# beecave-homelab/VibeVoice-ROCm

Hardware: AMD Instinct MI355X
Metric: audio-sec/s (higher is better)
Workload: dtype bf16; 1 GPU; cfg2: VibeVoice-1.5B shapes, 1 speaker(s) x 203-frame voice prompt, 330-token prompt, 225 frames (30.0 s audio), CFG=2.0, 20 DPM-Solver++ steps, whole generate() incl. voice encode + prefill; global_batch=1, parallelism=replicas x1 (one dialogue per GPU), hipgraph=True

## Files before the change

vibevoice_rocm_amd/csrc/vv_common.h:

```cpp
#ifndef VV_COMMON_H
#define VV_COMMON_H
#include <hip/hip_runtime.h>
#include <stdarg.h>
#include <stdint.h>
#include "vv_hip.h"

int vv_set_error(int code, const char* fmt, ...);

#define VV_CHECK_LAUNCH(name)                                                                    \
  do {                                                                                           \
    hipError_t e_ = hipGetLastError();                                                           \
    if (e_ != hipSuccess) return vv_set_error(VV_E_HIP, "%s: %s", name, hipGetErrorString(e_));  \
  } while (0)

#define VV_TRY(expr)            \
  do {                          \
    int rc_ = (expr);           \
    if (rc_) return rc_;        \
  } while (0)

struct vv_kv_args {
  void* k; void* v;
  int kvdt, layers, rows, kv_heads, s_max, head_dim;
  void* vt;
  vv_kv_args(const vv_kv& a) : k(a.k), v(a.v), kvdt(a.kvdt), layers(a.layers), rows(a.rows), kv_heads(a.kv_heads), s_max(a.s_max), head_dim(a.head_dim), vt(a.vt) {}
};
struct vv_kv_args8 : vv_kv_args {
  const float* kscale; const float* vscale;
  vv_kv_args8(const vv_kv& a) : vv_kv_args(a), kscale(a.kscale), vscale(a.vscale) {}
};

int vv_launch_gemv_stream(const vv_lin_args& a, hipStream_t s);
struct vv_gemv_hot_shape { const char* name; int m, n, k, dual, pro, mod, bias, gate, res, act, flags; };
extern "C" int vv_gemv_hot_shapes(vv_gemv_hot_shape* out, int cap);
int vv_launch_gemv_hot(const vv_lin_args& a, hipStream_t s);
void vv_gemv_hot_set(int mask);
int vv_launch_conv_hot_gemv(const vv_lin_args& a, hipStream_t s);
int vv_launch_conv_hot_row(const vv_block& B, const float* x, float* y, float* hidden, float* hist_new, int C, float eps, hipStream_t s);
void vv_conv_hot_set(int mask);
int vv_launch_gemv_rows(const vv_lin_args& a, float* part, size_t part_floats, int* tickets, size_t n_tickets, hipStream_t s);
size_t vv_gemv_rows_part_floats(int n, int dual);
size_t vv_gemv_rows_tickets(int n);
int vv_gemv_rows_init();
void vv_gemv_rows_set(int on, int blocks, int pers);
int vv_linear_ws(const vv_lin_args* a, const void* f1, const void* f2, float* part, size_t part_floats, int* tickets, size_t n_tickets,
                 vv_stream_t stream, const vv_w8* q1 = nullptr, const vv_w8* q2 = nullptr);
int vv_launch_mfma_gemm(const vv_lin_args& a, hipStream_t s);
int vv_mfma_gemm_init();
int vv_launch_attn_decode(const float* qkv, int64_t ld_qkv, int R, int heads, const vv_kv* kv, int layer, const float2* rope, const int* lens, float* out,
                          int64_t ldo, float* part, int* tickets, int nsplit, int part_cap, hipStream_t s);
int vv_attn_decode_ws(const float* qkv, int64_t ld_qkv, int R, int heads, const vv_kv* kv, int layer, const float* rope_table, const int* lens, float* out,
                      int64_t ldo, float* part, int* tickets, int nsplit, int part_cap, vv_stream_t stream);
int vv_launch_kv_quantize(const vv_kv* src, const vv_kv* dst, int src_row, int dst_row, int len, int flags, hipStream_t s);
int vv_launch_attn_prefill(const float* qkv, int64_t ld_qkv, int R, int heads, const vv_kv* kv, int layer, const int* lens, const int* cache_rows,
                           float* out, int64_t ldo, hipStream_t s);
int vv_head_init_fused(const vv_head* h, const float* noise, float* Xs, float* Ms, float* h0, int64_t ldh, hipStream_t s);
bool vv_head_boundary_supported(const vv_head* h);
int vv_head_boundary_fused(const vv_head* h, const float* hrows, int64_t ldh, const float* shift, const float* scale, int64_t ld_mod, float cfg,
                           const vv_dpm_coef* k, float* Xs, float* Ms, float* h_out, int64_t ldh_out, float* latent_out, hipStream_t s);
int vv_head_boundary_batch(const vv_head* h, const float* hrows, int64_t ldh, const float* shift, const float* scale, int64_t ld_mod, float cfg,
                           const vv_dpm_coef* k, float* Xs, float* Ms, int64_t state_stride, float* h_out, int64_t ldh_out, float* latent_out,
                           int64_t latent_stride, int B, hipStream_t s,
// ... 130 lines not shown
```

vibevoice_rocm_amd/csrc/vv_fused.hip:

```cpp
#include <hip/hip_runtime.h>
#include <stdint.h>

#include "vv_hip.h"
#include "vv_common.h"

namespace {

typedef unsigned short bf16_t;
__device__ __forceinline__ float bf2f(bf16_t v) { return __uint_as_float((unsigned)v << 16); }
__device__ __forceinline__ float ldw(const float* p) { return *p; }
__device__ __forceinline__ float ldw(const bf16_t* p) { return bf2f(*p); }

template <typename WT>
__global__ __launch_bounds__(256) void head_init_kernel(const WT* P, const float* noise, int D, int latent, float* Xs, float* Ms, float* h0, int64_t ldh) {
  extern __shared__ float nz[];
  for (int i = threadIdx.x; i < latent; i += blockDim.x) nz[i] = noise[i];
  __syncthreads();
  const int n = blockIdx.x * blockDim.x + threadIdx.x;
  if (n >= D + latent) return;
  float s;
  if (n < D) {
    s = 0.f;
    const WT* pr = P + (int64_t)n * latent;
    for (int j = 0; j < latent; ++j) s = fmaf(ldw(pr + j), nz[j], s);
// ... 146 lines not shown
    if (lane == 0) {
      const float x0 = a.k.alpha_s * xs_cur - a.k.sigma_s * z;
      float xt = a.k.cx * xs_cur - a.k.cd * x0;
      if (a.k.order == 2) xt -= 0.5f * a.k.cd * (a.k.rinv * (x0 - ms_cur));
      if constexpr (SDE) xt = fmaf(a.k.cn, nx_cur, xt);
      a.Xs[g] = xt;
      a.Ms[g] = x0;
      if (g < D) { a.h_out[g] = xt; a.h_out[a.ldh_out + g] = xt; }
      else a.latent_out[g - D] = xt;
    }
    g += gstride;
#pragma unroll
    for (int u = 0; u < KU; ++u) { cur[u][0] = nxt[u][0]; cur[u][1] = nxt[u][1]; }
    xs_cur = xs_nxt; ms_cur = ms_nxt;
    if constexpr (SDE) nx_cur = nx_nxt;
    if (g + gstride < N) {
      xs_nxt = a.Xs[g + gstride]; ms_nxt = a.Ms[g + gstride];
      if constexpr (SDE) nx_nxt = a.nx[g + gstride];
      issue(nxt, g + gstride);
    }
  }
}

template <int KU> void launch_boundary(const BoundaryArgs& a, int B, hipStream_t s) {
  const int n = a.D + a.latent;
  int blocks = (n + 3) / 4;
  if (blocks > 512) blocks = 512;
  if (B > 1 && blocks > 256) blocks = 256;
  if (a.nx) hipLaunchKernelGGL((head_boundary_kernel<KU, true>), dim3(blocks, B), dim3(256), 0, s, a);
  else hipLaunchKernelGGL((head_boundary_kernel<KU, false>), dim3(blocks, B), dim3(256), 0, s, a);
}

template <typename WT, bool SAMPLE>
__global__ __launch_bounds__(256) void llm_tail_kernel(const float* h, int64_t ldh, int R, int H, const float* norm_w, float eps, float* out, int64_t ldo,
                                                       const WT* w_valid, int nv, const int* ids, float* logits_out, int* token_out, const int* forced,
                                                       int* lens, int tok_start, int tok_diff, int* frame_ctr, const vv_sampler smp, const float* q) {
  extern __shared__ float hn0[];
  __shared__ float red[4];
  __shared__ float lg[16];
  const int tid = threadIdx.x, lane = tid & 63, wave = tid >> 6;
  for (int r = 0; r < R; ++r) {
    const float* xr = h + (int64_t)r * ldh;
    float s = 0.f;
    for (int c = tid; c < H; c += 256) { const float v = xr[c]; s = fmaf(v, v, s); }
    s = vv_wave_sum(s);
    __syncthreads();
    if (lane == 0) red[wave] = s;
    __syncthreads();
// ... 525 lines not shown
#pragma unroll
    for (int o = 0; o < 2; ++o)
#pragma unroll
      for (int r = 0; r < 2; ++r) c0[o][r] = vv_wave_sum(acc[o][r]);
#pragma unroll
    for (int ps = 0; ps < 2; ++ps) {
      const int i = lane + 64 * ps;
      if (i < a.n_steps) {
#pragma unroll
        for (int r = 0; r < 2; ++r) {
          const float v0 = c0[0][r] + te[ps][0], v1 = c0[1][r] + te[ps][1];
          const float s0 = v0 / (1.0f + expf(-v0)), s1 = v1 / (1.0f + expf(-v1));
          const unsigned u0 = __float_as_uint(s0), u1 = __float_as_uint(s1);
          const unsigned pk = ((u0 + 0x7fffu + ((u0 >> 16) & 1u)) >> 16) | (((u1 + 0x7fffu + ((u1 >> 16) & 1u)) >> 16) << 16);
          *reinterpret_cast<unsigned*>(a.c_out + ((int64_t)(i * 2 + r)) * D + n) = pk;
        }
      }
    }
  }
}

}

int vv_head_init_fused(const vv_head* h, const float* noise, float* Xs, float* Ms, float* h0, int64_t ldh, hipStream_t s) {
  const int n = h->D + h->latent;
  const int blocks = (n + 255) / 256;
  const size_t lds = (size_t)h->latent * sizeof(float);
  if (h->wdt == VV_F32) hipLaunchKernelGGL((head_init_kernel<float>), dim3(blocks), dim3(256), lds, s, (const float*)h->noisy_proj, noise, h->D, h->latent, Xs, Ms, h0, ldh);
  else hipLaunchKernelGGL((head_init_kernel<bf16_t>), dim3(blocks), dim3(256), lds, s, (const bf16_t*)h->noisy_proj, noise, h->D, h->latent, Xs, Ms, h0, ldh);
  VV_CHECK_LAUNCH("vv_head_init_fused");
  return 0;
}

int vv_head_sde_proj_fused(const vv_head* h, const float* sde_noise, int64_t ld_sde, int n_steps, int B, float* NX, hipStream_t s) {
  const int n = h->D + h->latent;
  const dim3 grid((n + 255) / 256, B * n_steps);
  const size_t lds = (size_t)h->latent * sizeof(float);
  if (h->wdt == VV_F32)
    hipLaunchKernelGGL((head_sde_proj_kernel<float>), grid, dim3(256), lds, s, (const float*)h->noisy_proj, sde_noise, ld_sde, n_steps, h->D, h->latent, NX);
  else
    hipLaunchKernelGGL((head_sde_proj_kernel<bf16_t>), grid, dim3(256), lds, s, (const bf16_t*)h->noisy_proj, sde_noise, ld_sde, n_steps, h->D, h->latent, NX);
  VV_CHECK_LAUNCH("vv_head_sde_proj_fused");
  return 0;
}

bool vv_head_boundary_supported(const vv_head* h) {
// ... 214 lines not shown
```

vibevoice_rocm_amd/csrc/vv_gemv_hot.hip:

```cpp
#include <hip/hip_runtime.h>
#include <stdint.h>

#include "vv_hip.h"
#include "vv_common.h"

namespace {

typedef unsigned short bf16_t;
typedef unsigned int u32x4 __attribute__((ext_vector_type(4)));
typedef float vf2 __attribute__((ext_vector_type(2)));

__device__ __forceinline__ float silu1(float v) { return v / (1.0f + expf(-v)); }

__device__ __forceinline__ void unpack8(const u32x4 v, float (&o)[8]) {
  o[0] = __uint_as_float(v.x << 16); o[1] = __uint_as_float(v.x & 0xffff0000u);
  o[2] = __uint_as_float(v.y << 16); o[3] = __uint_as_float(v.y & 0xffff0000u);
  o[4] = __uint_as_float(v.z << 16); o[5] = __uint_as_float(v.z & 0xffff0000u);
  o[6] = __uint_as_float(v.w << 16); o[7] = __uint_as_float(v.w & 0xffff0000u);
}

template <bool NT>
__device__ __forceinline__ u32x4 ldw(const bf16_t* p) {
  const u32x4* q = reinterpret_cast<const u32x4*>(p);
  if constexpr (NT) return __builtin_nontemporal_load(q);
  else return *q;
}

__device__ __forceinline__ void fma_unit(const u32x4 wv, const float (&x0)[8], const float (&x1)[8], vf2& p0, vf2& p1) {
  float w[8];
  unpack8(wv, w);
#pragma unroll
  for (int j = 0; j < 8; j += 2) p0 = __builtin_elementwise_fma(vf2{w[j], w[j + 1]}, vf2{x0[j], x0[j + 1]}, p0);
#pragma unroll
  for (int j = 0; j < 8; j += 2) p1 = __builtin_elementwise_fma(vf2{w[j], w[j + 1]}, vf2{x1[j], x1[j + 1]}, p1);
}

__device__ __forceinline__ float vv_hot_gate_res(float v, float g, float r) {
#pragma clang fp contract(off)
  const float t = v * g;
  return t + r;
}

#define VV_FENCE4(v) asm volatile("" : "+v"((v).x), "+v"((v).y), "+v"((v).z), "+v"((v).w))

template <int N, bool MOD, bool NT>
__global__ __launch_bounds__(256, 2) void hot_dual_kernel(const vv_lin_args a) {
  constexpr int K = 1536, KU = 3, M = 2, T = 256, NCH = 2, NCHUNKS = K / 4;
  constexpr int WAVES = 512 * 4, G = (N + WAVES - 1) / WAVES;
  constexpr bool RAGGED = (N % WAVES) != 0;
  __shared__ float red[4 * M];
  __shared__ __attribute__((aligned(16))) float xs[M * KU * 512];
  const int tid = threadIdx.x, lane = tid & 63;
  const int wave = __builtin_amdgcn_readfirstlane(tid >> 6);
  const int gw = wave * 512 + (int)blockIdx.x;
  const bf16_t* __restrict__ W = reinterpret_cast<const bf16_t*>(a.w);
  const bf16_t* __restrict__ W2 = reinterpret_cast<const bf16_t*>(a.w2);

  float4 xv[M][NCH], nv[NCH], sv[M][NCH], cv[M][NCH];
#pragma unroll
  for (int c = 0; c < NCH; ++c) {
    const int ch = tid + c * T;
    const int kk = ch < NCHUNKS ? ch * 4 : 0;
#pragma unroll
    for (int m = 0; m < M; ++m) xv[m][c] = *reinterpret_cast<const float4*>(a.x + (int64_t)m * a.ldx + kk);
    nv[c] = *reinterpret_cast<const float4*>(a.norm_w + kk);
    if constexpr (MOD) {
#pragma unroll
      for (int m = 0; m < M; ++m) {
        const int64_t mo = (int64_t)m * a.ld_mod + kk;
        sv[m][c] = *reinterpret_cast<const float4*>(a.mod_shift + mo);
        cv[m][c] = *reinterpret_cast<const float4*>(a.mod_scale + mo);
      }
    }
  }
  u32x4 wq[G][KU], wq2[G][KU];
#pragma unroll
  for (int i = 0; i < G; ++i) {
    const int n = gw + i * WAVES;
    const bool live = !RAGGED || i < G - 1 || n < N;
    const int off = live ? n * K + lane * 8 : 0;
#pragma unroll
    for (int u = 0; u < KU; ++u) {
      wq[i][u] = ldw<NT>(W + off + (live ? u * 512 : 0));
      wq2[i][u] = ldw<NT>(W2 + off + (live ? u * 512 : 0));
    }
  }
  __builtin_amdgcn_sched_barrier(0);
#pragma unroll
  for (int c = 0; c < NCH; ++c) {
#pragma unroll
    for (int m = 0; m < M; ++m) VV_FENCE4(xv[m][c]);
    VV_FENCE4(nv[c]);
    if constexpr (MOD) {
#pragma unroll
      for (int m = 0; m < M; ++m) { VV_FENCE4(sv[m][c]); VV_FENCE4(cv[m][c]); }
    }
  }

  float ss[M];
#pragma unroll
  for (int m = 0; m < M; ++m) {
    float s1 = 0.f;
#pragma unroll
    for (int c = 0; c < NCH; ++c) {
      const float4 v = xv[m][c];
      s1 += (tid + c * T < NCHUNKS) ? (v.x * v.x + v.y * v.y) + (v.z * v.z + v.w * v.w) : 0.f;
    }
    ss[m] = vv_wave_sum(s1);
  }
  if (lane == 0) {
#pragma unroll
    for (int m = 0; m < M; ++m) red[wave * M + m] = ss[m];
  }
  __syncthreads();
#pragma unroll
  for (int m = 0; m < M; ++m) {
    float tot = 0.f;
#pragma unroll
    for (int w4 = 0; w4 < 4; ++w4) tot += red[w4 * M + m];
    const float rstd = rsqrtf(tot / (float)a.k + a.eps);
#pragma unroll
    for (int c = 0; c < NCH; ++c) {
      const int ch = tid + c * T;
      float4 v = xv[m][c];
      v.x *= rstd; v.y *= rstd; v.z *= rstd; v.w *= rstd;
      v.x *= nv[c].x; v.y *= nv[c].y; v.z *= nv[c].z; v.w *= nv[c].w;
      if constexpr (MOD) {
        v.x = v.x * (1.0f + cv[m][c].x) + sv[m][c].x; v.y = v.y * (1.0f + cv[m][c].y) + sv[m][c].y;
        v.z = v.z * (1.0f + cv[m][c].z) + sv[m][c].z; v.w = v.w * (1.0f + cv[m][c].w) + sv[m][c].w;
      }
      if (ch < NCHUNKS) *reinterpret_cast<float4*>(&xs[(m * KU * 128 + ch) * 4]) = v;
    }
  }
  __syncthreads();
  float xr[M][KU][8];
#pragma unroll
  for (int m = 0; m < M; ++m)
#pragma unroll
    for (int u = 0; u < KU; ++u) {
      const float4 p = *reinterpret_cast<const float4*>(&xs[m * KU * 512 + u * 512 + lane * 8]);
      const float4 q = *reinterpret_cast<const float4*>(&xs[m * KU * 512 + u * 512 + lane * 8 + 4]);
      xr[m][u][0] = p.x; xr[m][u][1] = p.y; xr[m][u][2] = p.z; xr[m][u][3] = p.w;
      xr[m][u][4] = q.x; xr[m][u][5] = q.y; xr[m][u][6] = q.z; xr[m][u][7] = q.w;
    }

#pragma unroll
  for (int i = 0; i < G; ++i) {
    const int n = gw + i * WAVES;
    if (RAGGED && i == G - 1 && n >= N) break;
    vf2 p[M] = {vf2{0.f, 0.f}, vf2{0.f, 0.f}}, p2[M] = {vf2{0.f, 0.f}, vf2{0.f, 0.f}};
#pragma unroll
    for (int u = 0; u < KU; ++u) {
      fma_unit(wq[i][u], xr[0][u], xr[1][u], p[0], p[1]);
      fma_unit(wq2[i][u], xr[0][u], xr[1][u], p2[0], p2[1]);
    }
    float acc[M], acc2[M];
#pragma unroll
    for (int m = 0; m < M; ++m) {
      acc[m] = vv_wave_sum(p[m].x + p[m].y);
      acc2[m] = vv_wave_sum(p2[m].x + p2[m].y);
    }
    if (lane < M) {
      const float v = lane == 0 ? acc[0] : acc[1], v2 = lane == 0 ? acc2[0] : acc2[1];
      a.out[(int64_t)lane * a.ldo + n] = silu1(v) * v2;
    }
  }
}

template <int N, int WPB, bool RMS, bool NT>
__global__ __launch_bounds__(64 * WPB) void hot_rows_kernel(const vv_lin_args a) {
  constexpr int K = 1536, KU = 3, M = 2, RW = 2;
  static_assert(N % (RW * WPB) == 0, "every wave of the grid owns one whole row pair");
  const int tid = threadIdx.x, lane = tid & 63;
  const int wave = __builtin_amdgcn_readfirstlane(tid >> 6);
  const int g = (int)blockIdx.x * WPB + wave;
  const bf16_t* __restrict__ W = reinterpret_cast<const bf16_t*>(a.w);

  float4 xa[M][KU], xb[M][KU], na[KU], nb[KU];
#pragma unroll
  for (int m = 0; m < M; ++m) {
    const float* xrow = a.x + (int64_t)m * a.ldx + lane * 8;
#pragma unroll
    for (int u = 0; u < KU; ++u) {
      xa[m][u] = *reinterpret_cast<const float4*>(xrow + u * 512);
      xb[m][u] = *reinterpret_cast<const float4*>(xrow + u * 512 + 4);
    }
  }
  if constexpr (RMS) {
#pragma unroll
    for (int u = 0; u < KU; ++u) {
      na[u] = *reinterpret_cast<const float4*>(a.norm_w + u * 512 + lane * 8);
      nb[u] = *reinterpret_cast<const float4*>(a.norm_w + u * 512 + lane * 8 + 4);
    }
  }
  const int eo_id = lane < RW * M ? lane : 0;
  const int eo_r = eo_id >> 1, eo_m = eo_id & 1;
  const int eo_n = g * RW + eo_r;
  float eo;
  if constexpr (RMS) eo = a.bias[eo_n];
  else eo = a.res[(int64_t)eo_m * a.ldres + eo_n];
  u32x4 wq[RW][KU];
#pragma unroll
  for (int r = 0; r < RW; ++r)
#pragma unroll
    for (int u = 0; u < KU; ++u) wq[r][u] = ldw<NT>(W + (g * RW + r) * K + u * 512 + lane * 8);
  __builtin_amdgcn_sched_barrier(0);
#pragma unroll
  for (int u = 0; u < KU; ++u) {
#pragma unroll
    for (int m = 0; m < M; ++m) { VV_FENCE4(xa[m][u]); VV_FENCE4(xb[m][u]); }
    if constexpr (RMS) { VV_FENCE4(na[u]); VV_FENCE4(nb[u]); }
  }

  float xr[M][KU][8];
  float ss[M];
#pragma unroll
  for (int m = 0; m < M; ++m) {
    ss[m] = 0.f;
#pragma unroll
    for (int u = 0; u < KU; ++u) {
      xr[m][u][0] = xa[m][u].x; xr[m][u][1] = xa[m][u].y; xr[m][u][2] = xa[m][u].z; xr[m][u][3] = xa[m][u].w;
      xr[m][u][4] = xb[m][u].x; xr[m][u][5] = xb[m][u].y; xr[m][u][6] = xb[m][u].z; xr[m][u][7] = xb[m][u].w;
      if constexpr (RMS) {
#pragma unroll
        for (int j = 0; j < 8; ++j) ss[m] = fmaf(xr[m][u][j], xr[m][u][j], ss[m]);
      }
    }
  }
  if constexpr (RMS) {
#pragma unroll
    for (int m = 0; m < M; ++m) ss[m] = vv_wave_sum(ss[m]);
#pragma unroll
    for (int m = 0; m < M; ++m) {
      const float rstd = rsqrtf(ss[m] / (float)a.k + a.eps);
// ... 12 lines not shown

  vf2 p[RW][M];
#pragma unroll
  for (int r = 0; r < RW; ++r) {
    p[r][0] = vf2{0.f, 0.f}; p[r][1] = vf2{0.f, 0.f};
#pragma unroll
    for (int u = 0; u < KU; ++u) fma_unit(wq[r][u], xr[0][u], xr[1][u], p[r][0], p[r][1]);
  }
  float acc[RW][M];
#pragma unroll
  for (int r = 0; r < RW; ++r)
#pragma unroll
    for (int m = 0; m < M; ++m) acc[r][m] = vv_wave_sum(p[r][m].x + p[r][m].y);
  if (lane < RW * M) {
    const float v0 = (lane & 1) ? acc[0][1] : acc[0][0], v1 = (lane & 1) ? acc[1][1] : acc[1][0];
    float v = (lane & 2) ? v1 : v0;
    v += eo;
    a.out[(int64_t)eo_m * a.ldo + eo_n] = v;
  }
}

template <int N, int K, int R, bool GATE, bool NT>
__global__ __launch_bounds__(256) void hot_down_kernel(const vv_lin_args a) {
  constexpr int M = 2, NW = 4, UNITS = (K + 511) / 512, KU = (UNITS + NW - 1) / NW;
  static_assert(N % R == 0 && R * M <= 64, "whole row sets; the epilogue threads are the first R * M of the block");
  __shared__ float part[NW][R * M];
  const int tid = threadIdx.x, lane = tid & 63;
  const int wave = __builtin_amdgcn_readfirstlane(tid >> 6);
  const int n0 = (int)blockIdx.x * R;
  const bf16_t* __restrict__ W = reinterpret_cast<const bf16_t*>(a.w);

  int koff[KU];
  bool kval[KU];
#pragma unroll
  for (int u = 0; u < KU; ++u) {
    koff[u] = (wave + NW * u) * 512 + lane * 8;
    kval[u] = koff[u] < K;
    if (!kval[u]) koff[u] = 0;
  }
  float4 xa[M][KU], xb[M][KU];
#pragma unroll
  for (int m = 0; m < M; ++m) {
    const float* xrow = a.x + (int64_t)m * a.ldx;
#pragma unroll
    for (int u = 0; u < KU; ++u) {
      xa[m][u] = *reinterpret_cast<const float4*>(xrow + koff[u]);
// ... 7 lines not shown
  if constexpr (GATE) eg = a.gate[(int64_t)eo_m * a.gate_ld + eo_n];
  const float er = a.res[(int64_t)eo_m * a.ldres + eo_n];
  u32x4 wq[R][KU];
#pragma unroll
  for (int r = 0; r < R; ++r)
#pragma unroll
    for (int u = 0; u < KU; ++u) wq[r][u] = ldw<NT>(W + (n0 + r) * K + koff[u]);
  __builtin_amdgcn_sched_barrier(0);
#pragma unroll
  for (int u = 0; u < KU; ++u)
#pragma unroll
    for (int m = 0; m < M; ++m) { VV_FENCE4(xa[m][u]); VV_FENCE4(xb[m][u]); }

  float xr[M][KU][8];
#pragma unroll
  for (int m = 0; m < M; ++m)
#pragma unroll
    for (int u = 0; u < KU; ++u) {
      const bool kv = kval[u];
      xr[m][u][0] = kv ? xa[m][u].x : 0.f; xr[m][u][1] = kv ? xa[m][u].y : 0.f; xr[m][u][2] = kv ? xa[m][u].z : 0.f; xr[m][u][3] = kv ? xa[m][u].w : 0.f;
      xr[m][u][4] = kv ? xb[m][u].x : 0.f; xr[m][u][5] = kv ? xb[m][u].y : 0.f; xr[m][u][6] = kv ? xb[m][u].z : 0.f; xr[m][u][7] = kv ? xb[m][u].w : 0.f;
    }

  float acc[R][M];
#pragma unroll
  for (int r = 0; r < R; ++r) {
    vf2 p0 = vf2{0.f, 0.f}, p1 = vf2{0.f, 0.f};
#pragma unroll
    for (int u = 0; u < KU; ++u) fma_unit(wq[r][u], xr[0][u], xr[1][u], p0, p1);
    acc[r][0] = vv_wave_sum(p0.x + p0.y);
    acc[r][1] = vv_wave_sum(p1.x + p1.y);
  }
  if (lane == 0) {
#pragma unroll
    for (int r = 0; r < R; ++r) { part[wave][r * M] = acc[r][0]; part[wave][r * M + 1] = acc[r][1]; }
  }
  __syncthreads();
  if (tid < R * M) {
    float s = 0.f;
#pragma unroll
    for (int w4 = 0; w4 < NW; ++w4) s += part[w4][tid];
    float v = s;
    if constexpr (GATE) v = vv_hot_gate_res(v, eg, er);
    else v += er;
    a.out[(int64_t)eo_m * a.ldo + eo_n] = v;
  }
}

#undef VV_FENCE4

constexpr int N_HOT = 6;
const vv_gemv_hot_shape g_table[N_HOT] = {
    {"head.gate_up", 2, 4608, 1536, 1, VV_PRO_RMSNORM, 1, 0, 0, 0, VV_ACT_SWIGLU, VV_LIN_W_REUSED},
    {"head.down",    2, 1536, 4608, 0, VV_PRO_NONE,    0, 0, 1, 1, VV_ACT_NONE,   VV_LIN_W_REUSED},
    {"llm.gate_up",  2, 8960, 1536, 1, VV_PRO_RMSNORM, 0, 0, 0, 0, VV_ACT_SWIGLU, 0},
    {"llm.down",     2, 1536, 8960, 0, VV_PRO_NONE,    0, 0, 0, 1, VV_ACT_NONE,   0},
    {"llm.qkv",      2, 2048, 1536, 0, VV_PRO_RMSNORM, 0, 1, 0, 0, VV_ACT_NONE,   0},
    {"llm.o",        2, 1536, 1536, 0, VV_PRO_NONE,    0, 0, 0, 1, VV_ACT_NONE,   0},
};

constexpr int HOT_DEFAULT = 0x3f;
int g_hot = HOT_DEFAULT;

bool matches(const vv_gemv_hot_shape& e, const vv_lin_args& a) {
  return a.m == e.m && a.n == e.n && a.k == e.k && a.wdt == VV_BF16 && (a.w2 != nullptr) == (e.dual != 0) && a.pro == e.pro &&
         (a.pro != VV_PRO_RMSNORM || a.norm_w != nullptr) && (a.mod_scale != nullptr) == (e.mod != 0) && (!e.mod || a.mod_shift != nullptr) &&
         (a.bias != nullptr) == (e.bias != 0) && (a.gate != nullptr) == (e.gate != 0) && (!e.gate || a.gate_ld != 0) &&
         (a.res != nullptr) == (e.res != 0) && a.act == e.act && a.flags == e.flags;
}

}

void vv_gemv_hot_set(int mask) { g_hot = mask < 0 ? HOT_DEFAULT : mask; }

extern "C" int vv_gemv_hot_shapes(vv_gemv_hot_shape* out, int cap) {
  for (int i = 0; i < N_HOT && i < cap; ++i) out[i] = g_table[i];
  return N_HOT;
}

int vv_launch_gemv_hot(const vv_lin_args& a, hipStream_t s) {
  if (!(g_hot & ((1 << N_HOT) - 1)) || a.m != 2 || a.wdt != VV_BF16) return 0;
  int id = -1;
  for (int i = 0; i < N_HOT; ++i)
    if ((g_hot >> i & 1) && matches(g_table[i], a)) { id = i; break; }
  const bool r3 = (g_hot & 256) != 0;
  switch (id) {
    case 0: hipLaunchKernelGGL((hot_dual_kernel<4608, true, false>), dim3(512), dim3(256), 0, s, a); return 1;
    case 1:
      if (r3) hipLaunchKernelGGL((hot_down_kernel<1536, 4608, 3, true, false>), dim3(512), dim3(256), 0, s, a);
      else hipLaunchKernelGGL((hot_down_kernel<1536, 4608, 6, true, false>), dim3(256), dim3(256), 0, s, a);
      return 1;
    case 2: hipLaunchKernelGGL((hot_dual_kernel<8960, false, true>), dim3(512), dim3(256), 0, s, a); return 1;
    case 3:
      if (r3) hipLaunchKernelGGL((hot_down_kernel<1536, 8960, 3, false, true>), dim3(512), dim3(256), 0, s, a);
      else hipLaunchKernelGGL((hot_down_kernel<1536, 8960, 6, false, true>), dim3(256), dim3(256), 0, s, a);
      return 1;
    case 4: hipLaunchKernelGGL((hot_rows_kernel<2048, 4, true, true>), dim3(256), dim3(256), 0, s, a); return 1;
    case 5: hipLaunchKernelGGL((hot_rows_kernel<1536, 3, false, true>), dim3(256), dim3(192), 0, s, a); return 1;
  }
  return 0;
}
```

vibevoice_rocm_amd/csrc/vv_kernels.hip:

```cpp
#include <hip/hip_runtime.h>
#include <hip/hip_bf16.h>
#include <stdint.h>
#include <stdio.h>
#include <string.h>
#include <math.h>

#include "vv_hip.h"
#include "vv_common.h"

static thread_local char g_err[512] = "";

int vv_set_error(int code, const char* fmt, ...) {
  va_list ap;
  va_start(ap, fmt);
  vsnprintf(g_err, sizeof(g_err), fmt, ap);
  va_end(ap);
  return code;
}

extern "C" const char* vv_last_error(void) { return g_err; }
extern "C" int vv_abi_version(void) { return 6; }
int vv_mixer_init();
extern "C" int vv_init(void) {
  VV_TRY(vv_mixer_init());
// ... 31 lines not shown
void vv_mfma_set_tiled_small_dual(int t);
void vv_mfma_set_tiled_small_k(int k);
void vv_mixer_set_rows(int on);
void vv_mfma_set_mt_prefill(int mt);
extern int g_attn_group;
void vv_attn_decode_set_gqa(int on);
void vv_attn_decode_set_gqa_keys(int k);
extern "C" int vv_tune(const char* key, int value) {
  if (key && !strcmp(key, "gemv_long_cap")) { vv_gemv_stream_set_long(value, 0); return 0; }
  if (key && !strcmp(key, "gemv_long_ku")) { vv_gemv_stream_set_long(0, value); return 0; }
  if (key && !strcmp(key, "gemv_blocks")) { vv_gemv_stream_set_blocks(value); return 0; }
  if (key && !strcmp(key, "gemv_waves")) { vv_gemv_stream_set_waves(value); return 0; }
  if (key && !strcmp(key, "gemv_rows")) { vv_gemv_rows_set(value, 0, -1); return 0; }
  if (key && !strcmp(key, "gemv_rows_blocks")) { vv_gemv_rows_set(-1, value, -1); return 0; }
  if (key && !strcmp(key, "gemv_rows_pers")) { vv_gemv_rows_set(-1, 0, value); return 0; }
  if (key && !strcmp(key, "gemv_rows_scratch")) return rows_scratch(value);
  if (key && !strcmp(key, "gemv_rows_dbg")) { vv_gemv_rows_set_dbg(value); return 0; }
  if (key && !strcmp(key, "gemv_rows_atomic")) { vv_gemv_rows_set_atomic(value); return 0; }
  if (key && !strcmp(key, "gemv_opt")) { vv_gemv_stream_set_opt(value); return 0; }
  if (key && !strcmp(key, "gemv_dual_rw")) { vv_gemv_stream_set_dual_rw(value); return 0; }
  if (key && !strcmp(key, "gemv_small_rw")) { vv_gemv_stream_set_small_rw(value); return 0; }
  if (key && !strcmp(key, "gemv_hot")) { vv_gemv_hot_set(value); return 0; }
  if (key && !strcmp(key, "conv_hot")) { vv_conv_hot_set(value); return 0; }
  if (key && !strcmp(key, "mixer_rows")) { vv_mixer_set_rows(value); return 0; }
  if (key && !strcmp(key, "block1d_fused")) { vv_block1d_set_fused(value); return 0; }
  if (key && !strcmp(key, "block1d_blocks")) { vv_block1d_set_blocks(value); return 0; }
  if (key && !strcmp(key, "convffn")) { vv_convffn_set(value); return 0; }
  if (key && !strcmp(key, "convffn_t1")) { vv_convffn_set_t1(value); return 0; }
  if (key && !strcmp(key, "convffn_t1hs")) { vv_convffn_set_t1hs(value); return 0; }
  if (key && !strcmp(key, "convffn_rows512")) { vv_convffn_set_rows(512, value); return 0; }
  if (key && !strcmp(key, "convffn_rows256")) { vv_convffn_set_rows(256, value); return 0; }
  if (key && !strcmp(key, "convffn_rows128")) { vv_convffn_set_rows(128, value); return 0; }
  if (key && !strcmp(key, "convffn_c128")) { vv_convffn_set_c128(value); return 0; }
  if (key && !strcmp(key, "skinny")) { vv_skinny_set(value, 0, 0); return 0; }
  if (key && !strcmp(key, "skinny_min_m")) { vv_skinny_set(1, value, 0); return 0; }
  if (key && !strcmp(key, "skinny_max_m")) { vv_skinny_set(1, 0, value); return 0; }
  if (key && !strcmp(key, "mfma_tiled_bk128")) { vv_mfma_set_tiled_bk128(value); return 0; }
  if (key && !strcmp(key, "attn_group")) { g_attn_group = value; return 0; }
  if (key && !strcmp(key, "attn_gqa")) { vv_attn_decode_set_gqa(value); return 0; }
  if (key && !strcmp(key, "attn_gqa_keys")) { vv_attn_decode_set_gqa_keys(value); return 0; }
  if (key && !strcmp(key, "mfma_tiled_small_k")) { vv_mfma_set_tiled_small_k(value); return 0; }
  if (key && !strcmp(key, "mfma_tiled_dual_bk64")) { vv_mfma_set_tiled_dual_bk64(value); return 0; }
  if (key && !strcmp(key, "mfma_tiled_small_dual")) { vv_mfma_set_tiled_small_dual(value); return 0; }
  if (key && !strcmp(key, "mfma_tiled_small")) { vv_mfma_set_tiled_small(value); return 0; }
  if (key && !strcmp(key, "mfma_tiled_rows")) { vv_mfma_set_tiled_rows(value); return 0; }
  if (key && !strcmp(key, "mfma_mt")) { vv_mfma_set_mt(value); return 0; }
// ... 1645 lines not shown
```

Measured before the change: 42.99 audio-sec/s.

## Add 8-wave boundary kernel and contiguous row mapping for hot dual GEMV

Adds a specialized 512-thread diffusion-head boundary kernel for D=1536, B=1 with no noise. In it, four staging waves compute the RMS/modulated CFG input into LDS while the other four waves only prefetch weights, and each wave owns one output row. This kernel is enabled by default. The hot dual GEMV is refactored into a body with optional wave-split (W8), weight-first load ordering (WF) and a contiguous per-wave row mapping (CM, on by default), plus off-by-default QKV load-order and LDS variants and timing probes. The aim is to issue weight loads earlier and improve memory locality and latency hiding in the small decode GEMVs; the cost is a larger kernel zoo and higher register pressure.

```diff
diff --git a/vibevoice_rocm_amd/csrc/vv_common.h b/vibevoice_rocm_amd/csrc/vv_common.h
--- a/vibevoice_rocm_amd/csrc/vv_common.h
+++ b/vibevoice_rocm_amd/csrc/vv_common.h
@@ -38,6 +38,7 @@
 int vv_launch_conv_hot_gemv(const vv_lin_args& a, hipStream_t s);
 int vv_launch_conv_hot_row(const vv_block& B, const float* x, float* y, float* hidden, float* hist_new, int C, float eps, hipStream_t s);
 void vv_conv_hot_set(int mask);
+void vv_boundary_hot_set(int mask);
 int vv_launch_gemv_rows(const vv_lin_args& a, float* part, size_t part_floats, int* tickets, size_t n_tickets, hipStream_t s);
 size_t vv_gemv_rows_part_floats(int n, int dual);
 size_t vv_gemv_rows_tickets(int n);
diff --git a/vibevoice_rocm_amd/csrc/vv_fused.hip b/vibevoice_rocm_amd/csrc/vv_fused.hip
--- a/vibevoice_rocm_amd/csrc/vv_fused.hip
+++ b/vibevoice_rocm_amd/csrc/vv_fused.hip
@@ -192,8 +192,137 @@
   }
 }
 
+template <bool STAGE>
+__device__ __forceinline__ void boundary8_body(const BoundaryArgs& a, float* ys, float (*red)[2], const int tid, const int wave) {
+  constexpr int KU = 3, D = KU * 512, NCH = 2, NCHUNKS = D / 4;
+  const int lane = tid & 63;
+  const int N = D + a.latent;
+  const int g = (int)blockIdx.x * 8 + wave;
+  const bool live = g < N;
+  float4 hv[2][NCH], sv[2][NCH], cv[2][NCH];
+  if constexpr (STAGE) {
+#pragma unroll
+    for (int c = 0; c < NCH; ++c) {
+      const int ch = tid + c * 256;
+      const int kk = ch < NCHUNKS ? ch * 4 : 0;
+#pragma unroll
+      for (int r = 0; r < 2; ++r) hv[r][c] = *reinterpret_cast<const float4*>(a.h + r * a.ldh + kk);
+    }
+    __builtin_amdgcn_sched_barrier(0);
+  }
+  float4 gq[KU][2];
+#pragma unroll
+  for (int u = 0; u < KU; ++u) {
+    const int64_t off = live ? (int64_t)g * D + u * 512 + lane * 8 : 0;
+    gq[u][0] = *reinterpret_cast<const float4*>(a.G + off);
+    gq[u][1] = *reinterpret_cast<const float4*>(a.G + off + 4);
+  }
+  const float xs_cur = a.Xs[live ? g : 0], ms_cur = a.Ms[live ? g : 0];
+  if constexpr (STAGE) {
+    __builtin_amdgcn_sched_barrier(0);
+#pragma unroll
+    for (int c = 0; c < NCH; ++c) {
+      const int ch = tid + c * 256;
+      const int kk = ch < NCHUNKS ? ch * 4 : 0;
+#pragma unroll
+      for (int r = 0; r < 2; ++r) {
+        sv[r][c] = *reinterpret_cast<const float4*>(a.shift + r * a.ld_mod + kk);
+        cv[r][c] = *reinterpret_cast<const float4*>(a.scale + r * a.ld_mod + kk);
+      }
+    }
+  }
+  __builtin_amdgcn_sched_barrier(0);
+#define VV_FENCE4(v) asm volatile("" : "+v"((v).x), "+v"((v).y), "+v"((v).z), "+v"((v).w))
+  if constexpr (STAGE) {
+#pragma unroll
+    for (int c = 0; c < NCH; ++c)
+#pragma unroll
+      for (int r = 0; r < 2; ++r) VV_FENCE4(hv[r][c]);
+    float ss[2];
+#pragma unroll
+    for (int r = 0; r < 2; ++r) {
+      float s1 = 0.f;
+#pragma unroll
+      for (int c = 0; c < NCH; ++c) {
+        const float4 v = hv[r][c];
+        s1 += (tid + c * 256 < NCHUNKS) ? (v.x * v.x + v.y * v.y) + (v.z * v.z + v.w * v.w) : 0.f;
+      }
+      ss[r] = vv_wave_sum(s1);
+    }
+    if (lane == 0) { red[wave][0] = ss[0]; red[wave][1] = ss[1]; }
+  }
+  __syncthreads();
+  if constexpr (STAGE) {
+    __builtin_amdgcn_sched_barrier(0);
+#pragma unroll
+    for (int c = 0; c < NCH; ++c)
+#pragma unroll
+      for (int r = 0; r < 2; ++r) { VV_FENCE4(sv[r][c]); VV_FENCE4(cv[r][c]); }
+    const float rs0 = rsqrtf(((red[0][0] + red[1][0]) + (red[2][0] + red[3][0])) / (float)D + a.eps);
+    const float rs1 = rsqrtf(((red[0][1] + red[1][1]) + (red[2][1] + red[3][1])) / (float)D + a.eps);
+#pragma unroll
+    for (int c = 0; c < NCH; ++c) {
+      const int ch = tid + c * 256;
+      if (ch < NCHUNKS) {
+        const float4 h0 = hv[0][c], h1 = hv[1][c];
+        const float yc0 = h0.x * rs0 * (1.0f + cv[0][c].x) + sv[0][c].x, yu0 = h1.x * rs1 * (1.0f + cv[1][c].x) + sv[1][c].x;
+        const float yc1 = h0.y * rs0 * (1.0f + cv[0][c].y) + sv[0][c].y, yu1 = h1.y * rs1 * (1.0f + cv[1][c].y) + sv[1][c].y;
+        const float yc2 = h0.z * rs0 * (1.0f + cv[0][c].z) + sv[0][c].z, yu2 = h1.z * rs1 * (1.0f + cv[1][c].z) + sv[1][c].z;
+        const float yc3 = h0.w * rs0 * (1.0f + cv[0][c].w) + sv[0][c].w, yu3 = h1.w * rs1 * (1.0f + cv[1][c].w) + sv[1][c].w;
+        *reinterpret_cast<float4*>(&ys[ch * 4]) = make_float4(yu0 + a.cfg * (yc0 - yu0), yu1 + a.cfg * (yc1 - yu1), yu2 + a.cfg * (yc2 - yu2), yu3 + a.cfg * (yc3 - yu3));
+      }
+    }
+  }
+#undef VV_FENCE4
+  __syncthreads();
+  if constexpr (!STAGE) __builtin_amdgcn_sched_barrier(0);
+  float yr[KU][8];
+#pragma unroll
+  for (int u = 0; u < KU; ++u) {
+    const float4 p = *reinterpret_cast<const float4*>(&ys[u * 512 + lane * 8]);
+    const float4 q = *reinterpret_cast<const float4*>(&ys[u * 512 + lane * 8 + 4]);
+    yr[u][0] = p.x; yr[u][1] = p.y; yr[u][2] = p.z; yr[u][3] = p.w; yr[u][4] = q.x; yr[u][5] = q.y; yr[u][6] = q.z; yr[u][7] = q.w;
+  }
+  if (!live) return;
+  float acc = 0.f;
+#pragma unroll
+  for (int u = 0; u < KU; ++u) {
+    const float w[8] = {gq[u][0].x, gq[u][0].y, gq[u][0].z, gq[u][0].w, gq[u][1].x, gq[u][1].y, gq[u][1].z, gq[u][1].w};
+#pragma unroll
+    for (int j = 0; j < 8; ++j) acc = fmaf(w[j], yr[u][j], acc);
+  }
+  const float z = vv_wave_sum(acc);
+  if (lane == 0) {
+    const float x0 = a.k.alpha_s * xs_cur - a.k.sigma_s * z;
+    float xt = a.k.cx * xs_cur - a.k.cd * x0;
+    if (a.k.order == 2) xt -= 0.5f * a.k.cd * (a.k.rinv * (x0 - ms_cur));
+    a.Xs[g] = xt;
+    a.Ms[g] = x0;
+    if (g < D) { a.h_out[g] = xt; a.h_out[a.ldh_out + g] = xt; }
+    else a.latent_out[g - D] = xt;
+  }
+}
+
+__global__ __launch_bounds__(512) void head_boundary8_kernel(const BoundaryArgs a) {
+  __shared__ __attribute__((aligned(16))) float ys[3 * 512];
+  __shared__ float red[4][2];
+  const int tid = threadIdx.x;
+  const int wave = __builtin_amdgcn_readfirstlane(tid >> 6);
+  if (wave < 4) boundary8_body<true>(a, ys, red, tid, wave);
+  else boundary8_body<false>(a, ys, red, tid, wave);
+}
+
+constexpr int BOUNDARY_HOT_DEFAULT = 1;
+int g_boundary_hot = BOUNDARY_HOT_DEFAULT;
+
 template <int KU> void launch_boundary(const BoundaryArgs& a, int B, hipStream_t s) {
   const int n = a.D + a.latent;
+  if constexpr (KU == 3) {
+    if ((g_boundary_hot & 1) && a.D == 1536 && B == 1 && !a.nx) {
+      hipLaunchKernelGGL(head_boundary8_kernel, dim3((n + 7) / 8), dim3(512), 0, s, a);
+      return;
+    }
+  }
   int blocks = (n + 3) / 4;
   if (blocks > 512) blocks = 512;
   if (B > 1 && blocks > 256) blocks = 256;
@@ -765,6 +894,8 @@
 
 }
 
+void vv_boundary_hot_set(int mask) { g_boundary_hot = mask < 0 ? BOUNDARY_HOT_DEFAULT : mask; }
+
 int vv_head_init_fused(const vv_head* h, const float* noise, float* Xs, float* Ms, float* h0, int64_t ldh, hipStream_t s) {
   const int n = h->D + h->latent;
   const int blocks = (n + 255) / 256;
diff --git a/vibevoice_rocm_amd/csrc/vv_gemv_hot.hip b/vibevoice_rocm_amd/csrc/vv_gemv_hot.hip
--- a/vibevoice_rocm_amd/csrc/vv_gemv_hot.hip
+++ b/vibevoice_rocm_amd/csrc/vv_gemv_hot.hip
@@ -43,26 +43,38 @@
 
 #define VV_FENCE4(v) asm volatile("" : "+v"((v).x), "+v"((v).y), "+v"((v).z), "+v"((v).w))
 
-template <int N, bool MOD, bool NT>
-__global__ __launch_bounds__(256, 2) void hot_dual_kernel(const vv_lin_args a) {
+#ifdef VV_CF_TIMING
+__device__ unsigned long long g_hot_t[2][2];
+#define HSTAMP(kind, i) do { if (blockIdx.x == 0 && threadIdx.x == 0) { const long long t_ = wall_clock64(); g_hot_t[kind][i] += (unsigned long long)(t_ - tprev_); tprev_ = t_; } } while (0)
+#define HSTAMP_BEGIN long long tprev_ = wall_clock64()
+#else
+#define HSTAMP(kind, i) do { } while (0)
+#define HSTAMP_BEGIN do { } while (0)
+#endif
+
+template <int N, bool MOD, bool NT, bool WF, bool CM, bool STAGE>
+__device__ __forceinline__ void hot_dual_body(const vv_lin_args& a, float* red, float* xs, const int tid, const int wave, const int gw) {
+  HSTAMP_BEGIN;
   constexpr int K = 1536, KU = 3, M = 2, T = 256, NCH = 2, NCHUNKS = K / 4;
   constexpr int WAVES = 512 * 4, G = (N + WAVES - 1) / WAVES;
   constexpr bool RAGGED = (N % WAVES) != 0;
-  __shared__ float red[4 * M];
-  __shared__ __attribute__((aligned(16))) float xs[M * KU * 512];
-  const int tid = threadIdx.x, lane = tid & 63;
-  const int wave = __builtin_amdgcn_readfirstlane(tid >> 6);
-  const int gw = wave * 512 + (int)blockIdx.x;
+  constexpr int FULL = RAGGED ? G - 1 : G;
+  const int lane = tid & 63;
+  const int cm0 = ((gw & 511) * 4 + (gw >> 9)) * FULL;
+  auto row = [&](int i) { return CM && i < FULL ? cm0 + i : gw + i * WAVES; };
   const bf16_t* __restrict__ W = reinterpret_cast<const bf16_t*>(a.w);
   const bf16_t* __restrict__ W2 = reinterpret_cast<const bf16_t*>(a.w2);
 
   float4 xv[M][NCH], nv[NCH], sv[M][NCH], cv[M][NCH];
-#pragma unroll
-  for (int c = 0; c < NCH; ++c) {
+  auto load_x = [&](int c) {
     const int ch = tid + c * T;
     const int kk = ch < NCHUNKS ? ch * 4 : 0;
 #pragma unroll
     for (int m = 0; m < M; ++m) xv[m][c] = *reinterpret_cast<const float4*>(a.x + (int64_t)m * a.ldx + kk);
+  };
+  auto load_ops = [&](int c) {
+    const int ch = tid + c * T;
+    const int kk = ch < NCHUNKS ? ch * 4 : 0;
     nv[c] = *reinterpret_cast<const float4*>(a.norm_w + kk);
     if constexpr (MOD) {
 #pragma unroll
@@ -72,11 +84,19 @@
         cv[m][c] = *reinterpret_cast<const float4*>(a.mod_scale + mo);
       }
     }
+  };
+  if constexpr (STAGE) {
+#pragma unroll
+    for (int c = 0; c < NCH; ++c) {
+      load_x(c);
+      if constexpr (!WF) load_ops(c);
+    }
+    if constexpr (WF) __builtin_amdgcn_sched_barrier(0);
   }
   u32x4 wq[G][KU], wq2[G][KU];
 #pragma unroll
   for (int i = 0; i < G; ++i) {
-    const int n = gw + i * WAVES;
+    const int n = row(i);
     const bool live = !RAGGED || i < G - 1 || n < N;
     const int off = live ? n * K + lane * 8 : 0;
 #pragma unroll
@@ -85,54 +105,77 @@
       wq2[i][u] = ldw<NT>(W2 + off + (live ? u * 512 : 0));
     }
   }
+  if constexpr (STAGE && WF) {
+    __builtin_amdgcn_sched_barrier(0);
+#pragma unroll
+    for (int c = 0; c < NCH; ++c) load_ops(c);
+  }
   __builtin_amdgcn_sched_barrier(0);
-#pragma unroll
-  for (int c = 0; c < NCH; ++c) {
-#pragma unroll
-    for (int m = 0; m < M; ++m) VV_FENCE4(xv[m][c]);
-    VV_FENCE4(nv[c]);
-    if constexpr (MOD) {
-#pragma unroll
-      for (int m = 0; m < M; ++m) { VV_FENCE4(sv[m][c]); VV_FENCE4(cv[m][c]); }
-    }
-  }
-
-  float ss[M];
-#pragma unroll
-  for (int m = 0; m < M; ++m) {
-    float s1 = 0.f;
+
+  if constexpr (STAGE) {
 #pragma unroll
     for (int c = 0; c < NCH; ++c) {
-      const float4 v = xv[m][c];
-      s1 += (tid + c * T < NCHUNKS) ? (v.x * v.x + v.y * v.y) + (v.z * v.z + v.w * v.w) : 0.f;
-    }
-    ss[m] = vv_wave_sum(s1);
-  }
-  if (lane == 0) {
-#pragma unroll
-    for (int m = 0; m < M; ++m) red[wave * M + m] = ss[m];
+#pragma unroll
+      for (int m = 0; m < M; ++m) VV_FENCE4(xv[m][c]);
+      if constexpr (!WF) {
+        VV_FENCE4(nv[c]);
+        if constexpr (MOD) {
+#pragma unroll
+          for (int m = 0; m < M; ++m) { VV_FENCE4(sv[m][c]); VV_FENCE4(cv[m][c]); }
+        }
+      }
+    }
+    float ss[M];
+#pragma unroll
+    for (int m = 0; m < M; ++m) {
+      float s1 = 0.f;
+#pragma unroll
+      for (int c = 0; c < NCH; ++c) {
+        const float4 v = xv[m][c];
+        s1 += (tid + c * T < NCHUNKS) ? (v.x * v.x + v.y * v.y) + (v.z * v.z + v.w * v.w) : 0.f;
+      }
+      ss[m] = vv_wave_sum(s1);
+    }
+    if (lane == 0) {
+#pragma unroll
+      for (int m = 0; m < M; ++m) red[wave * M + m] = ss[m];
+    }
   }
   __syncthreads();
-#pragma unroll
-  for (int m = 0; m < M; ++m) {
-    float tot = 0.f;
-#pragma unroll
-    for (int w4 = 0; w4 < 4; ++w4) tot += red[w4 * M + m];
-    const float rstd = rsqrtf(tot / (float)a.k + a.eps);
-#pragma unroll
-    for (int c = 0; c < NCH; ++c) {
-      const int ch = tid + c * T;
-      float4 v = xv[m][c];
-      v.x *= rstd; v.y *= rstd; v.z *= rstd; v.w *= rstd;
-      v.x *= nv[c].x; v.y *= nv[c].y; v.z *= nv[c].z; v.w *= nv[c].w;
-      if constexpr (MOD) {
-        v.x = v.x * (1.0f + cv[m][c].x) + sv[m][c].x; v.y = v.y * (1.0f + cv[m][c].y) + sv[m][c].y;
-        v.z = v.z * (1.0f + cv[m][c].z) + sv[m][c].z; v.w = v.w * (1.0f + cv[m][c].w) + sv[m][c].w;
-      }
-      if (ch < NCHUNKS) *reinterpret_cast<float4*>(&xs[(m * KU * 128 + ch) * 4]) = v;
+  if constexpr (STAGE) {
+    if constexpr (WF) {
+      __builtin_amdgcn_sched_barrier(0);
+#pragma unroll
+      for (int c = 0; c < NCH; ++c) {
+        VV_FENCE4(nv[c]);
+        if constexpr (MOD) {
+#pragma unroll
+          for (int m = 0; m < M; ++m) { VV_FENCE4(sv[m][c]); VV_FENCE4(cv[m][c]); }
+        }
+      }
+    }
+#pragma unroll
+    for (int m = 0; m < M; ++m) {
+      float tot = 0.f;
+#pragma unroll
+      for (int w4 = 0; w4 < 4; ++w4) tot += red[w4 * M + m];
+      const float rstd = rsqrtf(tot / (float)a.k + a.eps);
+#pragma unroll
+      for (int c = 0; c < NCH; ++c) {
+        const int ch = tid + c * T;
+        float4 v = xv[m][c];
+        v.x *= rstd; v.y *= rstd; v.z *= rstd; v.w *= rstd;
+        v.x *= nv[c].x; v.y *= nv[c].y; v.z *= nv[c].z; v.w *= nv[c].w;
+        if constexpr (MOD) {
+          v.x = v.x * (1.0f + cv[m][c].x) + sv[m][c].x; v.y = v.y * (1.0f + cv[m][c].y) + sv[m][c].y;
+          v.z = v.z * (1.0f + cv[m][c].z) + sv[m][c].z; v.w = v.w * (1.0f + cv[m][c].w) + sv[m][c].w;
+        }
+        if (ch < NCHUNKS) *reinterpret_cast<float4*>(&xs[(m * KU * 128 + ch) * 4]) = v;
+      }
     }
   }
   __syncthreads();
+  if constexpr (!STAGE) __builtin_amdgcn_sched_barrier(0);
   float xr[M][KU][8];
 #pragma unroll
   for (int m = 0; m < M; ++m)
@@ -144,9 +187,13 @@
       xr[m][u][4] = q.x; xr[m][u][5] = q.y; xr[m][u][6] = q.z; xr[m][u][7] = q.w;
     }
 
+#ifdef VV_CF_TIMING
+  VV_FENCE4(wq[0][0]);
+  HSTAMP(0, 0);
+#endif
 #pragma unroll
   for (int i = 0; i < G; ++i) {
-    const int n = gw + i * WAVES;
+    const int n = row(i);
     if (RAGGED && i == G - 1 && n >= N) break;
     vf2 p[M] = {vf2{0.f, 0.f}, vf2{0.f, 0.f}}, p2[M] = {vf2{0.f, 0.f}, vf2{0.f, 0.f}};
 #pragma unroll
@@ -165,34 +212,64 @@
       a.out[(int64_t)lane * a.ldo + n] = silu1(v) * v2;
     }
   }
-}
-
-template <int N, int WPB, bool RMS, bool NT>
+  HSTAMP(0, 1);
+}
+
+template <int N, bool MOD, bool NT, bool WF, bool W8, bool CM>
+__global__ __launch_bounds__(W8 ? 512 : 256, W8 ? 1 : 2) void hot_dual_kernel(const vv_lin_args a) {
+  __shared__ float red[4 * 2];
+  __shared__ __attribute__((aligned(16))) float xs[2 * 3 * 512];
+  const int tid = threadIdx.x;
+  const int wave = __builtin_amdgcn_readfirstlane(tid >> 6);
+  if constexpr (W8) {
+    const int gw = (wave & 3) * 512 + (int)blockIdx.x + (wave >> 2) * 256;
+    if (wave < 4) hot_dual_body<N, MOD, NT, WF, CM, true>(a, red, xs, tid, wave, gw);
+    else hot_dual_body<N, MOD, NT, WF, CM, false>(a, red, xs, tid, wave, gw);
+  } else {
+    hot_dual_body<N, MOD, NT, WF, CM, true>(a, red, xs, tid, wave, wave * 512 + (int)blockIdx.x);
+  }
+}
+
+template <int N, int WPB, bool RMS, bool NT, int XM>
 __global__ __launch_bounds__(64 * WPB) void hot_rows_kernel(const vv_lin_args a) {
   constexpr int K = 1536, KU = 3, M = 2, RW = 2;
   static_assert(N % (RW * WPB) == 0, "every wave of the grid owns one whole row pair");
+  static_assert(XM == 0 || RMS, "the load-order variants are the RMSNorm prologue's");
+  static_assert(XM != 2 || WPB == 4, "a quarter of the 2 x 384 chunks per wave");
+  constexpr int XQ = M * (K / 4) / (4 * 64);
+  __shared__ __attribute__((aligned(16))) float xsh[XM == 2 ? M * K : 4];
   const int tid = threadIdx.x, lane = tid & 63;
   const int wave = __builtin_amdgcn_readfirstlane(tid >> 6);
   const int g = (int)blockIdx.x * WPB + wave;
   const bf16_t* __restrict__ W = reinterpret_cast<const bf16_t*>(a.w);
 
-  float4 xa[M][KU], xb[M][KU], na[KU], nb[KU];
-#pragma unroll
-  for (int m = 0; m < M; ++m) {
-    const float* xrow = a.x + (int64_t)m * a.ldx + lane * 8;
-#pragma unroll
-    for (int u = 0; u < KU; ++u) {
-      xa[m][u] = *reinterpret_cast<const float4*>(xrow + u * 512);
-      xb[m][u] = *reinterpret_cast<const float4*>(xrow + u * 512 + 4);
-    }
-  }
-  if constexpr (RMS) {
+  float4 xa[M][KU], xb[M][KU], na[KU], nb[KU], xq[XQ];
+  if constexpr (XM == 2) {
+#pragma unroll
+    for (int j = 0; j < XQ; ++j) {
+      const int q = wave * (XQ * 64) + j * 64 + lane, m = q / (K / 4), cc = q - m * (K / 4);
+      xq[j] = *reinterpret_cast<const float4*>(a.x + (int64_t)m * a.ldx + cc * 4);
+    }
+  } else {
+#pragma unroll
+    for (int m = 0; m < M; ++m) {
+      const float* xrow = a.x + (int64_t)m * a.ldx + lane * 8;
+#pragma unroll
+      for (int u = 0; u < KU; ++u) {
+        xa[m][u] = *reinterpret_cast<const float4*>(xrow + u * 512);
+        xb[m][u] = *reinterpret_cast<const float4*>(xrow + u * 512 + 4);
+      }
+    }
+  }
+  auto load_norm = [&]() {
 #pragma unroll
     for (int u = 0; u < KU; ++u) {
       na[u] = *reinterpret_cast<const float4*>(a.norm_w + u * 512 + lane * 8);
       nb[u] = *reinterpret_cast<const float4*>(a.norm_w + u * 512 + lane * 8 + 4);
     }
-  }
+  };
+  if constexpr (RMS && XM == 0) load_norm();
+  if constexpr (XM != 0) __builtin_amdgcn_sched_barrier(0);
   const int eo_id = lane < RW * M ? lane : 0;
   const int eo_r = eo_id >> 1, eo_m = eo_id & 1;
   const int eo_n = g * RW + eo_r;
@@ -204,12 +281,31 @@
   for (int r = 0; r < RW; ++r)
 #pragma unroll
     for (int u = 0; u < KU; ++u) wq[r][u] = ldw<NT>(W + (g * RW + r) * K + u * 512 + lane * 8);
+  if constexpr (RMS && XM != 0) {
+    __builtin_amdgcn_sched_barrier(0);
+    load_norm();
+  }
   __builtin_amdgcn_sched_barrier(0);
+  if constexpr (XM == 2) {
+#pragma unroll
+    for (int j = 0; j < XQ; ++j) {
+      VV_FENCE4(xq[j]);
+      *reinterpret_cast<float4*>(&xsh[(wave * (XQ * 64) + j * 64 + lane) * 4]) = xq[j];
+    }
+    __syncthreads();
+#pragma unroll
+    for (int m = 0; m < M; ++m)
+#pragma unroll
+      for (int u = 0; u < KU; ++u) {
+        xa[m][u] = *reinterpret_cast<const float4*>(&xsh[m * K + u * 512 + lane * 8]);
+        xb[m][u] = *reinterpret_cast<const float4*>(&xsh[m * K + u * 512 + lane * 8 + 4]);
+      }
+  }
 #pragma unroll
   for (int u = 0; u < KU; ++u) {
 #pragma unroll
     for (int m = 0; m < M; ++m) { VV_FENCE4(xa[m][u]); VV_FENCE4(xb[m][u]); }
-    if constexpr (RMS) { VV_FENCE4(na[u]); VV_FENCE4(nb[u]); }
+    if constexpr (RMS && XM == 0) { VV_FENCE4(na[u]); VV_FENCE4(nb[u]); }
   }
 
   float xr[M][KU][8];
@@ -268,6 +364,7 @@
 
 template <int N, int K, int R, bool GATE, bool NT>
 __global__ __launch_bounds__(256) void hot_down_kernel(const vv_lin_args a) {
+  HSTAMP_BEGIN;
   constexpr int M = 2, NW = 4, UNITS = (K + 511) / 512, KU = (UNITS + NW - 1) / NW;
   static_assert(N % R == 0 && R * M <= 64, "whole row sets; the epilogue threads are the first R * M of the block");
   __shared__ float part[NW][R * M];
@@ -321,6 +418,10 @@
       xr[m][u][4] = kv ? xb[m][u].x : 0.f; xr[m][u][5] = kv ? xb[m][u].y : 0.f; xr[m][u][6] = kv ? xb[m][u].z : 0.f; xr[m][u][7] = kv ? xb[m][u].w : 0.f;
     }
 
+#ifdef VV_CF_TIMING
+  VV_FENCE4(wq[0][0]);
+  HSTAMP(1, 0);
+#endif
   float acc[R][M];
 #pragma unroll
   for (int r = 0; r < R; ++r) {
@@ -344,6 +445,7 @@
     else v += er;
     a.out[(int64_t)eo_m * a.ldo + eo_n] = v;
   }
+  HSTAMP(1, 1);
 }
 
 #undef VV_FENCE4
@@ -358,8 +460,26 @@
     {"llm.o",        2, 1536, 1536, 0, VV_PRO_NONE,    0, 0, 0, 1, VV_ACT_NONE,   0},
 };
 
-constexpr int HOT_DEFAULT = 0x3f;
+constexpr int HOT_DUAL_WF = 1 << 9, HOT_DUAL_W8 = 1 << 10, HOT_QKV_WF = 1 << 11, HOT_QKV_LDS = 1 << 12, HOT_DUAL_CM = 1 << 13;
+constexpr int HOT_DEFAULT = 0x3f | HOT_DUAL_CM;
 int g_hot = HOT_DEFAULT;
+
+template <int N, bool MOD, bool NT, bool WF, bool W8>
+void launch_dual2(const vv_lin_args& a, hipStream_t s) {
+  if (g_hot & HOT_DUAL_CM) hipLaunchKernelGGL((hot_dual_kernel<N, MOD, NT, WF, W8, true>), dim3(W8 ? 256 : 512), dim3(W8 ? 512 : 256), 0, s, a);
+  else hipLaunchKernelGGL((hot_dual_kernel<N, MOD, NT, WF, W8, false>), dim3(W8 ? 256 : 512), dim3(W8 ? 512 : 256), 0, s, a);
+}
+template <int N, bool MOD, bool NT>
+void launch_dual(const vv_lin_args& a, hipStream_t s) {
+  const bool wf = (g_hot & HOT_DUAL_WF) != 0;
+  if (g_hot & HOT_DUAL_W8) {
+    if (wf) launch_dual2<N, MOD, NT, true, true>(a, s);
+    else launch_dual2<N, MOD, NT, false, true>(a, s);
+  } else {
+    if (wf) launch_dual2<N, MOD, NT, true, false>(a, s);
+    else launch_dual2<N, MOD, NT, false, false>(a, s);
+  }
+}
 
 bool matches(const vv_gemv_hot_shape& e, const vv_lin_args& a) {
   return a.m == e.m && a.n == e.n && a.k == e.k && a.wdt == VV_BF16 && (a.w2 != nullptr) == (e.dual != 0) && a.pro == e.pro &&
@@ -371,6 +491,14 @@
 }
 
 void vv_gemv_hot_set(int mask) { g_hot = mask < 0 ? HOT_DEFAULT : mask; }
+
+#ifdef VV_CF_TIMING
+extern "C" int vv_gemv_hot_debug_times(unsigned long long* out, int reset) {
+  hipError_t e = hipMemcpyFromSymbol(out, HIP_SYMBOL(g_hot_t), sizeof(unsigned long long) * 4);
+  if (e == hipSuccess && reset) { unsigned long long z[4] = {0, 0, 0, 0}; e = hipMemcpyToSymbol(HIP_SYMBOL(g_hot_t), z, sizeof(z)); }
+  return e == hipSuccess ? 0 : -1;
+}
+#endif
 
 extern "C" int vv_gemv_hot_shapes(vv_gemv_hot_shape* out, int cap) {
   for (int i = 0; i < N_HOT && i < cap; ++i) out[i] = g_table[i];
@@ -384,18 +512,22 @@
     if ((g_hot >> i & 1) && matches(g_table[i], a)) { id = i; break; }
   const bool r3 = (g_hot & 256) != 0;
   switch (id) {
-    case 0: hipLaunchKernelGGL((hot_dual_kernel<4608, true, false>), dim3(512), dim3(256), 0, s, a); return 1;
+    case 0: launch_dual<4608, true, false>(a, s); return 1;
     case 1:
       if (r3) hipLaunchKernelGGL((hot_down_kernel<1536, 4608, 3, true, false>), dim3(512), dim3(256), 0, s, a);
       else hipLaunchKernelGGL((hot_down_kernel<1536, 4608, 6, true, false>), dim3(256), dim3(256), 0, s, a);
       return 1;
-    case 2: hipLaunchKernelGGL((hot_dual_kernel<8960, false, true>), dim3(512), dim3(256), 0, s, a); return 1;
+    case 2: launch_dual<8960, false, true>(a, s); return 1;
     case 3:
       if (r3) hipLaunchKernelGGL((hot_down_kernel<1536, 8960, 3, false, true>), dim3(512), dim3(256), 0, s, a);
       else hipLaunchKernelGGL((hot_down_kernel<1536, 8960, 6, false, true>), dim3(256), dim3(256), 0, s, a);
       return 1;
-    case 4: hipLaunchKernelGGL((hot_rows_kernel<2048, 4, true, true>), dim3(256), dim3(256), 0, s, a); return 1;
-    case 5: hipLaunchKernelGGL((hot_rows_kernel<1536, 3, false, true>), dim3(256), dim3(192), 0, s, a); return 1;
+    case 4:
+      if (g_hot & HOT_QKV_LDS) hipLaunchKernelGGL((hot_rows_kernel<2048, 4, true, true, 2>), dim3(256), dim3(256), 0, s, a);
+      else if (g_hot & HOT_QKV_WF) hipLaunchKernelGGL((hot_rows_kernel<2048, 4, true, true, 1>), dim3(256), dim3(256), 0, s, a);
+      else hipLaunchKernelGGL((hot_rows_kernel<2048, 4, true, true, 0>), dim3(256), dim3(256), 0, s, a);
+      return 1;
+    case 5: hipLaunchKernelGGL((hot_rows_kernel<1536, 3, false, true, 0>), dim3(256), dim3(192), 0, s, a); return 1;
   }
   return 0;
 }
diff --git a/vibevoice_rocm_amd/csrc/vv_kernels.hip b/vibevoice_rocm_amd/csrc/vv_kernels.hip
--- a/vibevoice_rocm_amd/csrc/vv_kernels.hip
+++ b/vibevoice_rocm_amd/csrc/vv_kernels.hip
@@ -77,6 +77,7 @@
   if (key && !strcmp(key, "gemv_small_rw")) { vv_gemv_stream_set_small_rw(value); return 0; }
   if (key && !strcmp(key, "gemv_hot")) { vv_gemv_hot_set(value); return 0; }
   if (key && !strcmp(key, "conv_hot")) { vv_conv_hot_set(value); return 0; }
+  if (key && !strcmp(key, "boundary_hot")) { vv_boundary_hot_set(value); return 0; }
   if (key && !strcmp(key, "mixer_rows")) { vv_mixer_set_rows(value); return 0; }
   if (key && !strcmp(key, "block1d_fused")) { vv_block1d_set_fused(value); return 0; }
   if (key && !strcmp(key, "block1d_blocks")) { vv_block1d_set_blocks(value); return 0; }
```

Result: no change. 43.27 audio-sec/s, median of 6 (+0.7%).
